# QuentinHuan/ENSEM3A_OpenCLRaytracer

Measured on AMD Instinct MI355X. Metric: Msamples/s Cornell box 1024x1024 64spp; 1/2/4/8-GPU scaling; HBM %peak, higher is better.
Workload: dtype f32; 1 GPU; cornell_1024_s64; scene=cornell, width=1024, height=1024, spp=64, max_bounce=4, traversal=fast, bvh=sah, parallelism=row-interleaved x1

## Files before the change

### ensem3a_openclraytracer_amd/_native.py

```python
from __future__ import annotations

import ctypes
import os
import threading

import numpy as np

from ._build import LIB

_lock = threading.Lock()
_lib = None
_host = None

RT_TRAVERSAL_FAST = 0
RT_TRAVERSAL_REF = 1
RT_BVH_REFERENCE = 0
RT_BVH_SAH = 1
RT_ERR_ARG = 1
RT_ERR_STATE = 3
RT_ACCUM_MAX_SAMPLES = 1 << 24

EXPORTED = (
    "rt_create", "rt_destroy", "rt_last_error", "rt_set_scene", "rt_set_env", "rt_set_option",
    "rt_render", "rt_render_device", "rt_tile_rows", "rt_count_work", "rt_count_work_detail", "rt_work_bytes", "rt_gamma",
    "rt_render_rgb8", "rt_rgb8_device", "rt_rgb8",
    "rt_accum_begin", "rt_accum_add", "rt_accum_add_rgb8", "rt_accum_read", "rt_accum_samples", "rt_accum_end",
    "rt_accum_begin_device", "rt_accum_add_device",
    "rt_accum_mark", "rt_accum_select", "rt_accum_select_mask", "rt_accum_select_all", "rt_accum_selection",
    "rt_accum_sample_map", "rt_accum_add_selected", "rt_accum_mark_device", "rt_accum_select_device",
    "rt_accum_select_mask_device", "rt_accum_select_all_device", "rt_accum_add_selected_device",
    "rt_accum_guides", "rt_accum_guides_device", "rt_denoise_device", "rt_accum_denoise",
    "rt_trace", "rt_trace_device",
    "rt_bvh_build", "rt_device_count", "rt_debug_math", "rt_debug_fn", "rt_debug_trace", "rt_debug_trace_clustered", "rt_debug_scene_info", "rt_debug_pixel_log",
    "rt_debug_wave_counts", "rt_debug_quantise_axis", "rt_debug_timings", "rt_debug_brute_layout",
    "rt_debug_brute_clusters", "rt_debug_brute_shell", "rt_debug_brute_near", "rt_debug_brute_quad",
    "rt_debug_brute_direct", "rt_debug_last_direct", "rt_debug_shell_word",
    "rt_debug_brute_slices",
    "rt_debug_last_slices",
    "rt_debug_brute_refill", "rt_debug_last_refill", "rt_debug_last_launch",
    "rt_obj_parse", "rt_obj_size", "rt_obj_copy", "rt_obj_free", "rt_obj_last_error",
    "rt_scene_check", "rt_scene_last_error",
)
HOST_ONLY = ("rt_bvh_build", "rt_obj_parse", "rt_obj_size", "rt_obj_copy", "rt_obj_free", "rt_obj_last_error",
             "rt_scene_check", "rt_scene_last_error", "rt_debug_quantise_axis", "rt_debug_brute_layout",
             "rt_debug_brute_clusters", "rt_debug_brute_shell", "rt_debug_brute_near", "rt_debug_brute_quad")

_c_p = ctypes.c_void_p
_i64 = ctypes.c_int64
_i32 = ctypes.c_int


class DenoiseParams(ctypes.Structure):
    _fields_ = [("passes", ctypes.c_int), ("normal_squarings", ctypes.c_int),
                ("sigma_c", ctypes.c_float), ("sigma_p", ctypes.c_float)]
# ... 678 lines not shown
    return bool(out[0]), int(out[1]), int(out[2])


def last_slices() -> int:
    return int(lib().rt_debug_last_slices())


def brute_refill(nloc: int, lanes: int, option: int = -1) -> int:
    out = np.zeros(1, np.int32)
    st = lib().rt_debug_brute_refill(int(nloc), int(lanes), int(option), out.ctypes.data)
    if st != 0:
        raise NativeError(st, "rt_debug_brute_refill: bad arguments")
    return int(out[0])


def last_refill():
    out = np.zeros(3, np.int64)
    st = lib().rt_debug_last_refill(out.ctypes.data)
    if st != 0:
        raise NativeError(st, "rt_debug_last_refill: bad arguments")
    return int(out[0]), int(out[1]), int(out[2])


LAUNCH_FIELDS = ("trav", "count", "log", "smem", "ovf", "resume", "step", "wide", "brute", "ts", "acc",
                 "team", "walk_team", "slices", "refill", "grid", "lds", "shell", "near", "quad")
BRUTE_SLICED = 4
BRUTE_REFILL = 8


def last_launch() -> dict:
    out = np.zeros(len(LAUNCH_FIELDS), np.int32)
    st = lib().rt_debug_last_launch(out.ctypes.data)
    if st != 0:
        raise NativeError(st, "rt_debug_last_launch: bad arguments")
    return {name: int(v) for name, v in zip(LAUNCH_FIELDS, out)}


def tile_rows(npix: int, width: int, row0: int, row_step: int) -> int:
    return int(lib().rt_tile_rows(int(npix), int(width), int(row0), int(row_step)))
```

### ensem3a_openclraytracer_amd/csrc/rt_api.hip

```cpp
#include <hip/hip_runtime.h>

#include <cmath>
#include <cstdarg>
#include <cstdio>
#include <algorithm>
#include <array>
#include <atomic>
#include <chrono>
#include <cstring>
#include <map>
#include <string>
#include <thread>
#include <vector>

#include "../../include/rt_api.h"
#include "../../include/rt_debug.h"
#include "rt_internal.h"
#include "scene_pack.h"

constexpr int kResumeMinBvh2 = 36, kResumeMinWide = 48;
constexpr int kDenoiseLds = 1;

using rt::HostScene;

// ... 66 lines not shown
}

struct rt_ctx {
    std::vector<Device> devs;
    HostScene hs;
    bool have_scene = false;
    bool have_env = false;
    int ibl_w = 0, ibl_h = 0;
    int traversal = RT_TRAVERSAL_FAST;
    int bvh_layout = RT_BVH_SAH;
    int brute_max = RT_BRUTE_MAX_DEFAULT;
    int brute_cluster = -1;
    int brute_shell = -1;
    int brute_near = -1;
    int brute_direct = -1;
    int brute_quad = -1;
    int resume_min = -1;
    int team = 0;
    int walk_team = 0;
    int max_waves = 0;
    int step = 0;
    int sun_skip = 1;
    int sun_any = 1;
    int block = 128;
    int bvh_width = 0;
    int fixed_point = 1;
    int sun_cache = 1;
    int pilot = -1;
    int pilot_chunk = 0;
    int pilot_levels = 0;
// ... 144 lines not shown
    s.nmat = ctx->hs.nmat;
    s.ibl_sum = (const uint32_t*)d.ibl_sum.p;
    s.ibl_w = ctx->ibl_w;
    s.ibl_h = ctx->ibl_h;
    s.depth = wide ? std::max(ctx->hs.depth, ctx->hs.wdepth) : ctx->hs.depth;
    s.brute = (const float4*)d.brute.p;
    s.brute_box = (const float4*)d.brute_box.p;
    s.nbrute = ctx->hs.nbrute;
    s.nbox = ctx->hs.nbox;
    s.brute_cbox = (const float4*)d.brute_cbox.p;
    s.brute_crow = (const float4*)d.brute_crow.p;
    s.ncluster = ctx->hs.ncluster;
    s.ncslot = (int32_t)(ctx->hs.brute_cbox.size() / 8);
    s.nsingle4 = s.ncslot - rt::kClusterSlots * s.ncluster;
    s.host_flags = (ctx->brute_cluster < 0 ? rt::kHostClusterAuto : 0) | (ctx->hs.nquad > 0 ? rt::kHostQuad : 0) |
                   (ctx->hs.nshell > 0 && ctx->brute_direct != 0 ? rt::kHostDirect : 0);
    s.nsingle = ctx->hs.nsingle;
    s.shell = ctx->hs.nshell > 0 ? 2 * s.ncslot : 0;
    s.near_floor = s.shell && ctx->brute_near != 0 ? ctx->hs.shell_floor : 0.0f;
    s.near_mask_lo = s.near_floor != 0.0f ? (uint32_t)ctx->hs.shell_mask : 0u;
    s.near_mask_hi = s.near_floor != 0.0f ? (uint32_t)(ctx->hs.shell_mask >> 32) : 0u;
    s.stack_lds = std::min<int32_t>(s.depth > 0 ? s.depth : 1,
                                    ctx->stack_lds > 0 ? ctx->stack_lds : wide ? rt::kStackLdsWide : rt::kStackLds);
    s.stack_ovf = (int2*)d.stack_ovf.p;
    return s;
}

int check_frame(rt_ctx* ctx, const float* cam, const float* env, int64_t npix, int spp, int max_bounce, int row0,
                int row_step, rt::FrameParams* fp) {
    if (!ctx) return set_err(nullptr, RT_ERR_ARG, "null context");
    if (!ctx->have_scene) return set_err(ctx, RT_ERR_STATE, "rt_set_scene has not been called");
// ... 108 lines not shown
};

std::string bounds_message(const char* fmt, int a, int b = 0) {
    char buf[128];
    snprintf(buf, sizeof buf, fmt, a, b);
    return buf;
}

const std::vector<Option>& options() {
    constexpr Effect none = Effect::kNone, invalidate = Effect::kInvalidate, repack = Effect::kRepack;
    static const std::vector<Option> table = {
        {"traversal", &rt_ctx::traversal, range(RT_TRAVERSAL_FAST, RT_TRAVERSAL_REF), "traversal must be 0 (fast) or 1 (ref)", invalidate},
        {"brute_near", &rt_ctx::brute_near, range(-1, 1), "brute_near must be -1 (auto), 0 (off) or 1 (auto)", none},
        {"brute_quad", &rt_ctx::brute_quad, range(-1, 1), "brute_quad must be -1 (auto), 0 (off) or 1 (auto)", repack},
        {"brute_direct", &rt_ctx::brute_direct, range(-1, 1), "brute_direct must be -1 (auto), 0 (off) or 1 (auto)", repack},
        {"bvh", &rt_ctx::bvh_layout, range(RT_BVH_REFERENCE, RT_BVH_SAH), "bvh must be 0 (reference tree) or 1 (sah)", repack},
        {"brute_cluster", &rt_ctx::brute_cluster, range(-1, 1), "brute_cluster must be -1 (auto), 0 (off) or 1 (force)", repack},
        {"brute_shell", &rt_ctx::brute_shell, range(-1, 1), "brute_shell must be -1 (auto), 0 (off) or 1 (force)", repack},
        {"brute_max", &rt_ctx::brute_max, range(0, 4096), "brute_max must be in 0..4096", repack},
        {"resume_min", &rt_ctx::resume_min, range(-1, 64), "resume_min must be -1 (auto) or 0..64", none},
        {"team", &rt_ctx::team, one_of({0, 1, 2, 4, 8}), "team must be 0 (auto), 1, 2, 4 or 8", none},
        {"walk_team", &rt_ctx::walk_team, one_of({0, 1, 2, 4, 8}), "walk_team must be 0 (auto), 1, 2, 4 or 8", none},
        {"sun_any", &rt_ctx::sun_any, range(0, 1), "sun_any must be 0 or 1", none},
        {"sun_skip", &rt_ctx::sun_skip, range(0, 1), "sun_skip must be 0 or 1", none},
        {"step", &rt_ctx::step, range(0, 2), "step must be 0 (auto), 1 (item) or 2 (round)", none},
        {"waves", &rt_ctx::max_waves, range(0, 8), "waves must be in 0..8", none},
        {"pilot", &rt_ctx::pilot, range(-1, 1 << 20), "pilot must be -1 (auto), 0 (off) or a sample count", none},
        {"pilot_chunk", &rt_ctx::pilot_chunk, range(0, 4096), "pilot_chunk must be in 0..4096 (0 = auto)", none},
        {"pilot_levels", &rt_ctx::pilot_levels, zero_or(2, 256), "pilot_levels must be 0 (auto) or 2..256", none},
        {"stack_lds", &rt_ctx::stack_lds, zero_or(kStackLdsMin, rt::kStackLds),
// ... 1266 lines not shown
    const rt::LaunchNote n = rt::last_launch();
    const rt::KernelKey& k = n.key;
    const int64_t v[20] = {k.trav, k.count, k.log,  k.smem,       k.ovf,    k.resume, k.step, k.wide,          k.brute,
                           k.ts,   k.acc,   n.team, n.walk_team,  n.slices, n.refill, n.grid, (int64_t)n.lds,
                           n.shell, n.near, n.quad};
    for (int i = 0; i < 20; ++i) out[i] = (int32_t)std::min<int64_t>(v[i], INT32_MAX);
    return RT_OK;
}

int rt_debug_brute_refill(int64_t nloc, int64_t lanes, int option, int32_t* out) {
    if (!out || nloc < 0 || lanes < 0 || option < -1 || option > rt::kRefillMax) return RT_ERR_ARG;
    *out = rt::brute_refill_launch(option, nloc, lanes);
    return RT_OK;
}

int rt_debug_last_refill(int64_t out[3]) {
    if (!out) return RT_ERR_ARG;
    out[0] = rt::last_launch().refill;
    out[1] = g_refill_events.load(std::memory_order_relaxed);
    out[2] = g_refill_lanes.load(std::memory_order_relaxed);
    return RT_OK;
}

int rt_debug_timings(rt_ctx* ctx, double out[4]) {
    if (!ctx || !out) return set_err(ctx, RT_ERR_ARG, "bad arguments");
    out[0] = ctx->t_pack_ms;
    out[1] = ctx->t_upload_ms;
    out[2] = ctx->t_env_ms;
    out[3] = ctx->t_render_ms;
    return RT_OK;
// ... 17 lines not shown
```

### ensem3a_openclraytracer_amd/csrc/rt_internal.h

```cpp
#pragma once
#include <hip/hip_runtime.h>
#include <cstdint>

#include "rt_layout.h"
#include "rt_slices.h"

namespace rt {

constexpr int32_t kHostClusterAuto = 1;
constexpr int32_t kHostDirect = 4;
constexpr int32_t kHostQuad = 2;
struct DevScene {
    const float4* nodes;
    int32_t nnodes;
    int32_t root_ref;
    const float4* wnodes;
    const float4* wleaves;
    int32_t wroot_ref;
    float wdq_omax;
    float root_box[6];
    const float* bvh9;
    int32_t nbvh9;
    int32_t ref_stack;
    const float4* tri_geo;
    const float4* tri_fast;
    const float4* tri_shade;
// ... 119 lines not shown
    int log;
    int smem;
    int ovf;
    int resume;
    int step;
    int wide;
    int brute;
    int ts;
    int acc;
};
inline bool operator==(const KernelKey& a, const KernelKey& b) {
    return a.trav == b.trav && a.count == b.count && a.log == b.log && a.smem == b.smem && a.ovf == b.ovf &&
           a.resume == b.resume && a.step == b.step && a.wide == b.wide && a.brute == b.brute && a.ts == b.ts &&
           a.acc == b.acc;
}
KernelKey choose_kernel(const DevScene& sc, const FrameParams& fp, int traversal, bool count, bool log, int acc,
                        int block);
int64_t resident_blocks(const void* fn, int block, size_t lds, int max_waves, hipError_t* err);
struct QueryOptions {
    int engine;
    int grid_cap;
    int resume_min;
    int max_waves;
    int block;
};
hipError_t launch_query(const DevScene& sc, int traversal, int any, const float4* rays, float4* out, int64_t n,
                        const QueryOptions& q, unsigned int* counter, hipStream_t stream);
struct LaunchNote {
    KernelKey key;
    int team, walk_team, slices, refill;
// ... 31 lines not shown
```

### ensem3a_openclraytracer_amd/csrc/rt_kernels.hip

```cpp
#include <mutex>
#include <vector>

#include "rt_device.h"

namespace rt {

namespace {

__device__ __forceinline__ void save_state(float4* __restrict__ st, int p, rtm_f3 acc, float kc, uint32_t seed0,
                                           uint32_t seed1, int tc, int s) {
    st[2 * (int64_t)p] = make_float4(acc.x, acc.y, acc.z, kc);
    st[2 * (int64_t)p + 1] =
        make_float4(__uint_as_float(seed0), __uint_as_float(seed1), __int_as_float(tc), __int_as_float(s));
}

[[maybe_unused]] constexpr int kAccAdd = 1;
constexpr int kAccListed = 2;
constexpr int kBruteSliced = 4;
constexpr int kBruteRefill = 8;
template <int TRAV, bool COUNT, bool LOG = false, bool SMEM = false, bool OVF = false, int BRUTE_ = 0, int ACC = 0>
#ifndef RT_RENDER_WAVES
#define RT_RENDER_WAVES 5
#endif
__global__ void __launch_bounds__(256) __attribute__((amdgpu_waves_per_eu(RT_RENDER_WAVES))) render_kernel(DevScene S, FrameParams F, float* __restrict__ out,
                                               unsigned long long* __restrict__ counts,
                                               unsigned int* __restrict__ work_counter,
                                               const LaunchConst* __restrict__ lconst) {
    constexpr int BRUTE = BRUTE_ & 3;
    constexpr bool SLICED = (BRUTE_ & kBruteSliced) != 0;
    static_assert(!SLICED || BRUTE == 1 || BRUTE == 3, "sample slices: the one-lane brute-force loops");
    constexpr bool kRefill = (BRUTE == 1 || BRUTE == 3) && ((BRUTE_ & kBruteRefill) != 0 || COUNT || LOG);
    static_assert(!(BRUTE_ & kBruteRefill) || BRUTE == 1 || BRUTE == 3, "refill threshold: the one-lane brute-force loops");
    extern __shared__ __attribute__((aligned(16))) int lds_stack[];
    const int B = blockDim.x;
    int* stk = lds_stack + threadIdx.x;
    const LaneStack lst = lane_stack(S, lds_stack);
    Cnt c{};
    const float4* mtrec = nullptr;
    const float4* boxrec = nullptr;
    const float4* tshade = S.tri_shade;
    const float4* tframe = S.tri_frame;
    const float* tmat = S.mat;
    constexpr bool ROWS = RT_SHADE_ROWS && (BRUTE == 1 || BRUTE == 3);
    const float4* trow = nullptr;
    if (BRUTE) {
        float4* lr = reinterpret_cast<float4*>(reinterpret_cast<char*>(lds_stack) + (B / 64) * BRUTE_WAVE_LDS);
        float4* ls = lr + 3 * S.nbrute;
// ... 56 lines not shown
    const int W = F.width;
    const int imgSize = (int)F.npix;
    const float e3 = F.env[3], e4 = F.env[4];
    const int spp = F.spp, maxB = F.max_bounce;
    const unsigned int nloc = ACC == kAccListed ? (unsigned int)__builtin_amdgcn_readfirstlane((int)*F.pilot_cost)
                                                : (unsigned int)F.nloc;
    const int lane = threadIdx.x & 63;
    const int ts = BRUTE == 2 ? F.team : 1;
    const int team_lane0 = lane & ~(ts - 1);
    const bool team_leader = lane == team_lane0;
    const unsigned long long team_leaders = ts == 1 ? ~0ull : ts == 2 ? 0x5555555555555555ull
                                             : ts == 4 ? 0x1111111111111111ull : 0x0101010101010101ull;

    int phase = FETCH;
    PixelQueue pq;
    pq.per = (F.handout && F.pass != 2) ? (unsigned)(((ACC == kAccListed ? (int64_t)nloc : F.nloc) + kGroups - 1) / kGroups) : 0u;
    if constexpr (kRefill) pq.dry = F.refill > 1 ? (unsigned)min(F.refill, 64) << kQueueRefillShift : 0u;
    int p = 0, i = 0;
    bool logme = false;
    uint32_t seed0 = 0, seed1 = 0;
    rtm_f3 cd = rtm_v3(0, 0, 0);
    float kc = 1000.0f;
    int tc = -1;
    rtm_f3 so = rtm_v3(1, 1, 1);
    float k = 1000.0f;
    int tri = -1, j = 0;
    rtm_f3 Bo = rtm_v3(0, 0, 0), Bd = rtm_v3(0, 0, 0);
    rtm_f3 acc = rtm_v3(0, 0, 0);
    int s = 0;
    [[maybe_unused]] int plim = 0;
    auto slimit = [&]() __attribute__((always_inline)) { if constexpr (ACC == kAccListed) return plim; else return spp; };
// ... 39 lines not shown
        }
        if (need) {
            unsigned sl = kWholeJob;
            unsigned int q;
            if constexpr (SLICED) q = take_job<kRefill>(pq, need, team_lane0, work_counter, nloc, lane, nsl, stail, sl);
            else q = take_pixel<kRefill>(pq, need, team_lane0, work_counter, nloc, lane);
            if (SLICED && phase == FETCH && q < nloc && sl != kWholeJob && sl > 0) {
                p = (int)q;
                lim = (int)sl;
                s = send(sl - 1u);
                phase = WAIT_SLICE;
            } else if (phase == FETCH) {
                const bool whole = !SLICED || sl == kWholeJob;
                bool ok = q < nloc;
                if (ok) {
                    p = (ACC == kAccListed || F.pass == 2) ? (int)F.pilot_order[q] : (int)q;
                    const int krow = p / W;
                    const int col = p - krow * W;
                    const int64_t i64 = ((int64_t)F.row0 + (int64_t)krow * F.row_step) * W + col;
                    ok = i64 < F.npix;
                    i = (int)i64;
                }
                if (ok) {
                    if constexpr (SLICED) {
                        seed0 = (uint32_t)i;
                        seed1 = 0;
                    } else {
                        seed0 = (uint32_t)(i % imgSize);
                        seed1 = (uint32_t)(i / imgSize);
                    }
                    cd = camera_dir(C, W, i);
                    acc = rtm_v3(0, 0, 0);
                    s = 0;
                    cost = 0;
                    sun0 = -2;
                    phase = PRIMARY;
                    logme = LOG && i == F.log_pixel;
                    if (F.pass == 2) {
                        const float4 a = F.pilot_state[2 * (int64_t)p], b = F.pilot_state[2 * (int64_t)p + 1];
                        acc = rtm_v3(a.x, a.y, a.z);
                        kc = a.w;
                        seed0 = __float_as_uint(b.x);
                        seed1 = __float_as_uint(b.y);
                        tc = __float_as_int(b.z);
                        s = __float_as_int(b.w);
                        tri = tc; j = 0;
                        so = rtm_v3(1, 1, 1);
                        phase = s >= spp ? FETCH : PREP;
                    }
                    if constexpr (ACC) if (ACC == kAccListed || F.pilot > 0) {
                        const float4 a = F.pilot_state[2 * (int64_t)p], b = F.pilot_state[2 * (int64_t)p + 1];
                        acc = rtm_v3(a.x, a.y, a.z);
                        kc = a.w;
// ... 25 lines not shown
                so = rtm_v3(1, 1, 1);
                lim = send((unsigned)lim);
                phase = s >= spp ? FETCH : PREP;
            }
        }
        if (__all(phase == DONE)) break;
        if (SLICED && __all(phase == DONE || phase == WAIT_SLICE)) __builtin_amdgcn_s_sleep(8);
        if (COUNT && lane == 0) c.wave_outer++;
        if (phase == DONE || phase == FETCH || (SLICED && phase == WAIT_SLICE)) continue;

        if (phase == PREP) {
            bool done = true;
            const bool cam = j == 0;
            const rtm_f3 Ro = cam ? C.position : Bo, Rd = cam ? cd : Bd;
            const float kh = cam ? kc : k;
            if (j > maxB) {
            } else if (tri < 0) {
                so = rtm_scale(rtm_mul(so, sample_ibl_if<COUNT>(S, C, Rd, e4, c)), e4);
            } else {
                const float4 sh = ROWS ? trow[2 * tri] : tshade[tri];
                const rtm_f3 n = xyz(sh);
                const Mat cm = ROWS ? row_mat(sh, trow[2 * tri + 1]) : load_mat(tmat, __float_as_int(sh.w));
                if (cm.type == 0) {
                    so = rtm_scale(so, cm.rough);
                } else {
                    const float4 f2 = tframe[3 * tri + 2];
                    const rtm_f3 nn = xyz(f2);
                    float invPdf = 0.0f;
                    rtm_f3 brdf = rtm_v3(0, 0, 0);
                    if (COUNT) count_event(c, cm.type);
                    if (cm.type == 1) {
// ... 10 lines not shown
                        invPdf = 1.0f / rtm_fabs(rtm_dot(Bd, nn));
                    }
                    const rtm_f3 nd = dev_normalize(Rd);
                    Bo = rtm_v3(fmaf(nd.x, kh, Ro.x), fmaf(nd.y, kh, Ro.y), fmaf(nd.z, kh, Ro.z));
                    const float att = invPdf * rtm_fabs(rtm_dot(Bd, nn));
                    so = rtm_scale(rtm_mul(so, brdf), att);
                    phase = BOUNCE;
                    done = false;
                }
            }
            if (done) {
                if (LOG && logme) log_event(F, 3.0f, s + 1, rtm_v3(0, 0, 0), rtm_v3(0, 0, 0), 0.0f, 0, so);
                acc = rtm_add(acc, so);
                if (COUNT) c.samples++;
                ++s;
                if (TRAV == TRAV_FAST && F.fixed_point && j == 0 && !(LOG && logme)) {
                    if (COUNT) c.samples += (unsigned long long)max(slimit() - s, 0);
                    for (; s < slimit(); ++s) acc = rtm_add(acc, so);
                }
                if (s >= slimit()) {
                    phase = FETCH;
                    if (team_leader) store_pixel(out, p, acc, slimit());
                    if (F.pass == 1) save_pilot();
                    if constexpr (ACC) { if (team_leader) save_state(F.pilot_state, p, acc, kc, seed0, seed1, tc, s); }
                    if constexpr (SLICED) { if (lim < spp) save_slice(cd); }
                } else if (F.pass == 1 && s >= F.pilot) {
                    save_pilot();
                    phase = FETCH;
                } else if (SLICED && s >= lim) {
                    save_slice(cd);
                    phase = FETCH;
                } else {
                    tri = tc; j = 0;
                    so = rtm_v3(1, 1, 1);
                }
                continue;
            }
        }

        const rtm_f3 to = (phase == PRIMARY) ? C.position : Bo;
        const rtm_f3 td = (phase == PRIMARY) ? cd : ((phase == BOUNCE) ? Bd : C.sun);
// ... 1 lines not shown
        if constexpr (STAMPS) chain_stamp(stamp_wl, kStampHead);
        const Hit h = trace<TRAV, COUNT, SMEM, OVF, BRUTE != 0, BRUTE == 3>(S, nodes, tris, to, td, stk, B, lst, c, mtrec, ts, boxrec);
        if (COUNT && lane == __ffsll((long long)__ballot(1)) - 1) {
            const unsigned long long dt = clock64() - t_tr;
            c.cyc_trav += dt;
            c.cyc_shade -= dt;
        }
        ++cost;
        bool finish = false;
        if (phase == PRIMARY) {
            tc = h.tri;
            kc = h.k;
            tri = tc; j = 0;
            so = rtm_v3(1, 1, 1);
            phase = PREP;
            if (spp <= 0) {
                if (team_leader) store_pixel(out, p, acc, spp);
                phase = FETCH;
            }
            continue;
        }
        if (LOG && logme) {
            const int hm = h.tri >= 0 ? __float_as_int(S.tri_shade[h.tri].w) : 0;
            log_event(F, phase == BOUNCE ? 1.0f : 2.0f, j, Bo, td, h.tri >= 0 ? h.k : -1.0f, hm, so);
        }
        int sun_hit = -2;
        const bool sun_first = TRAV == TRAV_FAST && F.sun_cache && j == 0 && !(LOG && logme);
        if (phase == BOUNCE) {
            if (h.tri >= 0) {
                tri = h.tri; k = h.k;
                const Mat bm = ROWS ? row_mat(trow[2 * h.tri], trow[2 * h.tri + 1])
                                    : load_mat(tmat, __float_as_int(tshade[h.tri].w));
                if (bm.type != 0) {
                    if (j == maxB) {
                        so = rtm_v3(0, 0, 0);
                        finish = true;
                    } else {
                        ++j;
                        phase = PREP;
                    }
                } else {
                    so = rtm_scale(so, bm.rough);
                    finish = true;
                }
            } else if (TRAV == TRAV_FAST && F.sun_skip) {
                sun_hit = -1;
            } else if (sun_first && sun0 != -2) {
                sun_hit = sun0;
            } else {
                phase = SUN;
            }
        } else {
            sun_hit = h.tri;
            if (sun_first) sun0 = h.tri;
        }
        if (sun_hit != -2) {
            rtm_f3 sunLight = rtm_v3(0, 0, 0);
            if (COUNT) c.sun++;
            const Mat cm = ROWS ? row_mat(trow[2 * tri], trow[2 * tri + 1])
                                : load_mat(tmat, __float_as_int(tshade[tri].w));
            if (sun_hit < 0 && cm.type != 3) sunLight = rtm_v3(e3, e3, e3);
            if (sun_hit >= 0) {
                const Mat sm = ROWS ? row_mat(trow[2 * sun_hit], trow[2 * sun_hit + 1])
                                    : load_mat(tmat, __float_as_int(tshade[sun_hit].w));
                if (sm.type == 3) sunLight = rtm_scale(sm.color, e3);
            }
            const rtm_f3 envLight = rtm_scale(sample_ibl_if<COUNT>(S, C, Bd, e4, c), e4);
            so = rtm_mul(so, rtm_add(sunLight, envLight));
            finish = true;
        }
        if (finish) {
            if (LOG && logme) log_event(F, 3.0f, s + 1, rtm_v3(0, 0, 0), rtm_v3(0, 0, 0), 0.0f, 0, so);
            acc = rtm_add(acc, so);
            if (COUNT) c.samples++;
            ++s;
            if (s >= slimit()) {
                if (team_leader) store_pixel(out, p, acc, slimit());
                if (F.pass == 1) save_pilot();
                if constexpr (ACC) { if (team_leader) save_state(F.pilot_state, p, acc, kc, seed0, seed1, tc, s); }
                phase = FETCH;
            } else if (F.pass == 1 && s >= F.pilot) {
                save_pilot();
                phase = FETCH;
            } else if (SLICED && s >= lim) {
                save_slice(cd);
                phase = FETCH;
            } else {
                tri = tc; j = 0;
                so = rtm_v3(1, 1, 1);
                phase = PREP;
            }
        }
    }
    if constexpr (STAMPS) {
        if ((threadIdx.x & 63) == 0 && counts) {
            const unsigned long long* st = reinterpret_cast<const unsigned long long*>(stamp_wl + BRUTE_STAMP_OFF);
// ... 502 lines not shown
    t.push_back(walk_row<COUNT, false, true, false, false, 0, 1>());
    t.push_back(walk_row<COUNT, false, false, true, false, 0, 1>());
    t.push_back(walk_row<COUNT, false, false, false, false, 0, 1>());
    t.push_back(render_row<TRAV_FAST, COUNT, false, false, false, 1>());
    if constexpr (!COUNT) t.push_back(render_row<TRAV_FAST, COUNT, false, false, false, 3>());
    t.push_back(render_row<TRAV_FAST, COUNT, false, false, false, 2>());
    if constexpr (!COUNT) t.push_back(render_row<TRAV_FAST, COUNT, false, false, false, 3 | kBruteSliced>());
    t.push_back(render_row<TRAV_FAST, COUNT, false, false, false, 1 | kBruteSliced>());
    if constexpr (!COUNT) {
        t.push_back(render_row<TRAV_FAST, COUNT, false, false, false, 3 | kBruteSliced | kBruteRefill>());
        t.push_back(render_row<TRAV_FAST, COUNT, false, false, false, 1 | kBruteSliced | kBruteRefill>());
        t.push_back(render_row<TRAV_FAST, COUNT, false, false, false, 3 | kBruteRefill>());
        t.push_back(render_row<TRAV_FAST, COUNT, false, false, false, 1 | kBruteRefill>());
    }
}

__global__ void debug_math_kernel(int fn, const float* __restrict__ x, const float* __restrict__ y,
                                  float* __restrict__ out, int64_t n) {
    const int64_t i = (int64_t)blockIdx.x * blockDim.x + threadIdx.x;
    if (i >= n) return;
    float r = 0.0f;
    switch (fn) {
        case 0: r = rtm_sin(x[i]); break;
        case 1: r = rtm_cos(x[i]); break;
        case 2: r = rtm_tan(x[i]); break;
        case 3: r = rtm_asin(x[i]); break;
        case 4: r = rtm_acos(x[i]); break;
        case 5: r = rtm_atan2(x[i], y[i]); break;
        case 6: r = sqrtf(x[i]); break;
        case 7: r = x[i] / y[i]; break;
// ... 161 lines not shown
#endif

namespace {
const void* kernel_fn(const KernelKey& k) {
    static const std::vector<KernelRow> table = [] {
        std::vector<KernelRow> t;
#ifndef RT_ACCUM_TU
        log_rows(t);
        head_rows<true>(t);
        head_rows<false>(t);
        engine_rows<true>(t);
#else
        head_rows<false>(t);
#endif
        engine_rows<false>(t);
        return t;
    }();
    for (const KernelRow& r : table)
        if (r.key == k) return r.fn;
    return nullptr;
}

hipError_t launch_pick(const DevScene& sc, const FrameParams& fp, KernelKey k, int block, float* d_out,
                       unsigned long long* d_counts, unsigned int* d_work, hipStream_t stream) {
    if (fp.nloc <= 0) return hipSuccess;
    const bool brute = k.brute != 0, product = !k.count && !k.log, listed = k.acc == kAccListed;
    size_t lds = (brute ? brute_lds_bytes(sc, block, true) : stack_lds_bytes(sc, k.trav, block)) +
                 (k.smem ? staged_scene_bytes(sc) : 0);
    hipError_t e = hipSuccess;
    auto resident = [&](int max_waves) { return resident_blocks(kernel_fn(k), block, lds, max_waves, &e); };
// ... 5 lines not shown
    if (brute && !listed && fp.pass == 0 && fp.team <= 1 && fp.slice_state && fp.slice_ready &&
        sc.ntri + 2 < 65536 && fp.npix <= INT_MAX)
        bslices = brute_slice_launch(fp.slices, fp.nloc, lanes);
    if (!k.resume) f.slices = bslices;
    f.team = !brute ? 1 : bslices ? 1 : fp.team;
    if (f.team == 0) f.team = (!listed && fp.nloc * 4 <= lanes) ? 4 : 1;
    f.walk_team = 1;
    if (k.resume && k.step && !k.wide && !k.log) {
        f.walk_team = fp.walk_team ? fp.walk_team : listed ? 1 : auto_walk_team(fp.nloc, lanes);
        if (f.walk_team != 2 && f.walk_team != 4 && f.walk_team != 8) f.walk_team = 1;
    }
    f.refill = (brute && f.team <= 1) ? brute_refill_launch(fp.refill, fp.nloc, lanes) : 0;
    k.ts = f.walk_team;
    if (brute && f.team > 1) k.brute = 2;
    else if (brute) k.brute |= (bslices ? kBruteSliced : 0) | (product && f.refill > 1 ? kBruteRefill : 0);
    if (brute && f.team <= 1) lds = brute_lds_bytes(sc, block, false);
    const void* fn = kernel_fn(k);
    const int64_t need = (fp.nloc * f.team * f.walk_team + block - 1) / block;
    const int64_t grid = std::min(need, resident(fp.max_waves));
    if (e != hipSuccess) return e;
    if (bslices) e = hipMemsetAsync(f.slice_ready, 0, (size_t)fp.nloc * sizeof(uint32_t), stream);
    const LaunchConst* lc = nullptr;
    if (e == hipSuccess) e = setup_work_block(f, d_work, stream, &lc);
    if (e != hipSuccess) return e;
    const int shell = (k.brute & 3) == 3 && sc.shell != 0;
    note_launch({k, f.team, f.walk_team, f.slices, f.refill, grid, lds, shell, shell && sc.near_floor != 0.0f,
                 shell && (sc.host_flags & kHostQuad) != 0, shell && (sc.host_flags & kHostDirect) != 0});
#if RT_CHAIN_STAMPS
    if (!d_counts) d_counts = chain_stamp_buffer();
#endif
// ... 424 lines not shown
```

### ensem3a_openclraytracer_amd/csrc/scene_pack.cpp

```cpp
#include "scene_pack.h"

#include <algorithm>
#include <array>
#include <cmath>
#include <cstdarg>
#include <cstdio>
#include <cstring>
#include <atomic>
#include <functional>
#include <map>
#include <mutex>
#include <new>
#include <stdexcept>
#include <string>
#include <system_error>
#include <thread>
#include <vector>

#include "../../include/rt_api.h"
#include "../../include/rt_debug.h"
#include "../../include/rt_scene.h"
#include "bvh_sah.h"

using rt::HostScene;
// ... 826 lines not shown
    emit_bvh(hs, L.data(), R.data(), T.data(), box.data(), nn);
    return true;
}

}

namespace rt {

bool shell_direct(HostScene& hs, int direct) {
    if (hs.nshell <= 0 || hs.brute_shell.size() < (size_t)rt::kShellRecF) return false;
    const int32_t w = as_i32(hs.brute_shell[7]);
    hs.brute_shell[7] = as_f32(direct != 0 ? (w | rt::kShellDirect) : (w & ~rt::kShellDirect));
    return direct != 0;
}

void pack_checked(HostScene& hs, const float* bvh9, int64_t nb, int64_t ntri, int layout, int brute_max, int cluster,
                  int shell, int quad, std::string& why) {
    hs.fast_ok = (ntri > 0) ? pack_fast(hs, bvh9, nb, ntri, layout, brute_max, cluster, shell, quad, why) : true;
    if (hs.fast_ok && ntri > 0) {
        double m1 = 0.0, m2 = 0.0;
        for (int64_t t = 0; t < ntri; ++t) {
            const float* g = hs.tri_geo.data() + 12 * t;
            const double l1 = std::sqrt((double)g[4] * g[4] + (double)g[5] * g[5] + (double)g[6] * g[6]);
            const double l2 = std::sqrt((double)g[8] * g[8] + (double)g[9] * g[9] + (double)g[10] * g[10]);
            if (std::isfinite(l1)) m1 = std::max(m1, l1);
            if (std::isfinite(l2)) m2 = std::max(m2, l2);
        }
        if (!(m1 * m2 <= std::ldexp(1.0, 120))) {
            hs.fast_ok = false;
            why = "triangle edges beyond 2^60 (the FAST reciprocal needs |e1 . (d x e2)| <= 2^126)";
// ... 38 lines not shown
    for (int64_t m = 0; m < M; ++m) {
        const float tf = mat[6 * m];
        if (!(tf > -1.0f && tf < 4.0f))
            return fail(msg, RT_ERR_SCENE, "material %lld has type %g; the kernel defines types 0..3", (long long)m,
                           (double)tf);
    }
    hs.ntri = (int32_t)T;
    hs.nmat = (int32_t)M;
    hs.nbvh9 = (int32_t)NB;
    hs.mat.assign((size_t)rt::kMatF * M, 0.0f);
    for (int64_t m = 0; m < M; ++m) {
        for (int k = 0; k < 6; ++k) hs.mat[(size_t)rt::kMatF * m + k] = mat[6 * m + k];
        for (int k = 1; k < 4; ++k) hs.colors_finite = hs.colors_finite && std::isfinite(mat[6 * m + k]);
        hs.has_glass = hs.has_glass || (int)mat[6 * m] == 3;
    }
    if (bvh9) hs.bvh9.assign(bvh9, bvh9 + nbvh);
    hs.tri_geo.assign((size_t)T * 12, 0.0f);
    hs.tri_shade.assign((size_t)T * 4, 0.0f);
    for (int64_t t = 0; t < T; ++t) {
        const int32_t* f = face + 10 * t;
        if (f[0] < 0 || f[0] >= M)
            return fail(msg, RT_ERR_ARG, "triangle %lld: material %d out of range [0,%lld)", (long long)t, f[0],
                           (long long)M);
        for (int j = 7; j < 10; ++j)
            if (f[j] < 0 || f[j] >= NV)
                return fail(msg, RT_ERR_ARG, "triangle %lld: position index %d out of range", (long long)t, f[j]);
        if (f[4] < 0 || f[4] >= NN)
            return fail(msg, RT_ERR_ARG, "triangle %lld: normal index %d out of range", (long long)t, f[4]);
        const float* a = vp + 3 * (int64_t)f[7];
        const float* b = vp + 3 * (int64_t)f[8];
// ... 284 lines not shown
```

### ensem3a_openclraytracer_amd/csrc/scene_pack.h

```cpp
#pragma once
#include <cstdint>
#include <string>
#include <vector>

#include "rt_layout.h"

namespace rt {

struct HostScene {
    std::vector<float> nodes;
    std::vector<float> wnodes;
    std::vector<float> wleaves;
    int32_t nwnodes = 0, wroot_ref = 0, wdepth = 1;
    float wdq_omax = 0.0f;
    std::vector<float> bvh9;
    std::vector<float> tri_geo;
    std::vector<float> tri_fast;
    std::vector<float> tri_shade;
    std::vector<float> mat;
    std::vector<float> brute;
    std::vector<float> brute_box;
    int32_t nbrute = 0;
    int32_t nbox = 0;
    std::vector<float> brute_cbox;
    std::vector<float> brute_crow;
    int32_t ncluster = 0, nsingle = 0;
    std::vector<float> brute_shell;
    int32_t nshell = 0, nrest = 0;
    int32_t nquad = 0;
    std::vector<uint8_t> brute_near;
    float shell_floor = 0.0f;
    uint64_t shell_mask = 0;
    int32_t nnodes = 0, root_ref = 0, ntri = 0, nmat = 0, nbvh9 = 0, depth = 1;
    float root_box[6] = {0, 0, 0, 0, 0, 0};
    bool fast_ok = false;
    bool colors_finite = true;
    bool has_glass = false;
};


int scene_prepare(HostScene& hs, const float* vp, int64_t nvp, const float* vn, int64_t nvn, const int32_t* face,
                  int64_t nface, const float* mat, int64_t nmat, const float* bvh9, int64_t nbvh, int layout,
                  int brute_max, int cluster, int shell, int quad, std::string& msg, std::string& why);

void pack_checked(HostScene& hs, const float* bvh9, int64_t nb, int64_t ntri, int layout, int brute_max, int cluster,
                  int shell, int quad, std::string& why);

bool shell_direct(HostScene& hs, int direct);

}
```

### include/rt_debug.h

```cpp
#ifndef RT_DEBUG_H
#define RT_DEBUG_H

#include <stdint.h>
#include "rt_api.h"


#ifdef __cplusplus
extern "C" {
#endif

int rt_debug_math(rt_ctx* ctx, int fn, const float* x, const float* y, float* out, int64_t n);

int rt_debug_trace(rt_ctx* ctx, int traversal, const float* rays, float* out, int64_t n);

int rt_debug_trace_clustered(rt_ctx* ctx, const float* rays, float* out, int64_t n, int32_t info[4]);

enum {
    RT_FN_CAMERA = 0, RT_FN_SUN = 1, RT_FN_HEMI = 2, RT_FN_GGX = 3, RT_FN_IBL = 4, RT_FN_MT_REF = 5,
    RT_FN_MT_FAST = 6, RT_FN_BOX_REF = 7, RT_FN_BOX_FAST = 8, RT_FN_COUNT = 9
};
int rt_debug_fn(rt_ctx* ctx, int fn, const float* in, float* out, int64_t n);

int rt_debug_pixel_log(rt_ctx* ctx, int traversal, const float cam[10], const float env[5], int64_t npix, int spp,
                       int max_bounce, int64_t pixel, float* log, int cap, int* n_events, float out3[3]);
// ... 35 lines not shown

int rt_debug_last_direct(void);

int rt_debug_shell_word(rt_ctx* ctx);

int rt_debug_brute_slices(int64_t nloc, int64_t lanes, int spp, int option, int accum_base, int32_t out[3]);

int rt_debug_last_slices(void);

int rt_debug_last_launch(int32_t out[20]);

int rt_debug_brute_refill(int64_t nloc, int64_t lanes, int option, int32_t* out);

int rt_debug_last_refill(int64_t out[3]);

#ifdef __cplusplus
}
#endif
#endif
```

Before: 12610 Msamples/s.

## Add lean brute-force kernel variant for diffuse-only scenes without IBL

Adds a compile-time LEAN flag to the one-lane brute-force render kernels, selected automatically when every material is diffuse or emissive, the environment-map weight is zero, and no pilot or accumulation passes are in use. The lean path skips IBL sampling, pilot-order indirection and pilot state saves, and most material loads, and reads the material type and colour straight from the row data. This cuts per-bounce work and register pressure but adds more kernel instantiations. It also relies on the host-side material classification to be correct for it to be safe.

```diff
diff --git a/ensem3a_openclraytracer_amd/_native.py b/ensem3a_openclraytracer_amd/_native.py
--- a/ensem3a_openclraytracer_amd/_native.py
+++ b/ensem3a_openclraytracer_amd/_native.py
@@ -37,7 +37,7 @@
     "rt_debug_brute_direct", "rt_debug_last_direct", "rt_debug_shell_word",
     "rt_debug_brute_slices",
     "rt_debug_last_slices",
-    "rt_debug_brute_refill", "rt_debug_last_refill", "rt_debug_last_launch",
+    "rt_debug_brute_refill", "rt_debug_last_refill", "rt_debug_last_launch", "rt_debug_brute_lean",
     "rt_obj_parse", "rt_obj_size", "rt_obj_copy", "rt_obj_free", "rt_obj_last_error",
     "rt_scene_check", "rt_scene_last_error",
 )
@@ -746,6 +746,21 @@
     return int(out[0])
 
 
+def brute_lean(materialData, env, spp: int = 4, max_bounce: int = 4, pass_: int = 0, pilot: int = 0,
+               fixed_point: int = 1, sun_cache: int = 1, option: int = -1, loop: int = 3, team: int = 1,
+               count: int = 0, log: int = 0, acc: int = 0, traversal: int = 0):
+    mat, e = f32(materialData), f32(env)
+    fn = lib().rt_debug_brute_lean
+    fn.restype, fn.argtypes = _i32, [_c_p, _i64, _c_p, _c_p, _c_p, _c_p]
+    frame = np.array([spp, max_bounce, pass_, pilot, fixed_point, sun_cache, option], np.int32)
+    kernel = np.array([loop, team, count, log, acc, traversal], np.int32)
+    out = np.zeros(2, np.int32)
+    st = fn(ptr(mat) if mat.size else None, mat.size, ptr(e), frame.ctypes.data, kernel.ctypes.data, out.ctypes.data)
+    if st != 0:
+        raise NativeError(st, "rt_debug_brute_lean: bad arguments")
+    return bool(out[0]), bool(out[1])
+
+
 def last_refill():
     out = np.zeros(3, np.int64)
     st = lib().rt_debug_last_refill(out.ctypes.data)
@@ -758,6 +773,7 @@
                  "team", "walk_team", "slices", "refill", "grid", "lds", "shell", "near", "quad")
 BRUTE_SLICED = 4
 BRUTE_REFILL = 8
+BRUTE_LEAN = 16
 
 
 def last_launch() -> dict:
diff --git a/ensem3a_openclraytracer_amd/csrc/rt_api.hip b/ensem3a_openclraytracer_amd/csrc/rt_api.hip
--- a/ensem3a_openclraytracer_amd/csrc/rt_api.hip
+++ b/ensem3a_openclraytracer_amd/csrc/rt_api.hip
@@ -104,6 +104,7 @@
     int brute_shell = -1;
     int brute_near = -1;
     int brute_direct = -1;
+    int brute_lean = -1;
     int brute_quad = -1;
     int resume_min = -1;
     int team = 0;
@@ -278,7 +279,8 @@
     s.ncslot = (int32_t)(ctx->hs.brute_cbox.size() / 8);
     s.nsingle4 = s.ncslot - rt::kClusterSlots * s.ncluster;
     s.host_flags = (ctx->brute_cluster < 0 ? rt::kHostClusterAuto : 0) | (ctx->hs.nquad > 0 ? rt::kHostQuad : 0) |
-                   (ctx->hs.nshell > 0 && ctx->brute_direct != 0 ? rt::kHostDirect : 0);
+                   (ctx->hs.nshell > 0 && ctx->brute_direct != 0 ? rt::kHostDirect : 0) |
+                   (ctx->hs.diffuse_only && ctx->brute_lean != 0 ? rt::kHostLean : 0);
     s.nsingle = ctx->hs.nsingle;
     s.shell = ctx->hs.nshell > 0 ? 2 * s.ncslot : 0;
     s.near_floor = s.shell && ctx->brute_near != 0 ? ctx->hs.shell_floor : 0.0f;
@@ -417,6 +419,7 @@
         {"brute_near", &rt_ctx::brute_near, range(-1, 1), "brute_near must be -1 (auto), 0 (off) or 1 (auto)", none},
         {"brute_quad", &rt_ctx::brute_quad, range(-1, 1), "brute_quad must be -1 (auto), 0 (off) or 1 (auto)", repack},
         {"brute_direct", &rt_ctx::brute_direct, range(-1, 1), "brute_direct must be -1 (auto), 0 (off) or 1 (auto)", repack},
+        {"brute_lean", &rt_ctx::brute_lean, range(-1, 1), "brute_lean must be -1 (auto), 0 (off) or 1 (auto)", none},
         {"bvh", &rt_ctx::bvh_layout, range(RT_BVH_REFERENCE, RT_BVH_SAH), "bvh must be 0 (reference tree) or 1 (sah)", repack},
         {"brute_cluster", &rt_ctx::brute_cluster, range(-1, 1), "brute_cluster must be -1 (auto), 0 (off) or 1 (force)", repack},
         {"brute_shell", &rt_ctx::brute_shell, range(-1, 1), "brute_shell must be -1 (auto), 0 (off) or 1 (force)", repack},
@@ -1713,6 +1716,24 @@
     return RT_OK;
 }
 
+int rt_debug_brute_lean(const float* mat, int64_t nmat6, const float env[5], const int32_t frame[7],
+                        const int32_t kernel[6], int32_t out[2]) {
+    if ((nmat6 > 0 && !mat) || nmat6 < 0 || nmat6 % 6 || !env || !frame || !kernel || !out) return RT_ERR_ARG;
+    if (frame[6] < -1 || frame[6] > 1) return RT_ERR_ARG;
+    out[0] = rt::materials_diffuse_only(mat, nmat6) ? 1 : 0;
+    rt::FrameParams fp{};
+    std::memcpy(fp.env, env, sizeof fp.env);
+    fp.spp = frame[0];
+    fp.max_bounce = frame[1];
+    fp.pass = frame[2];
+    fp.pilot = frame[3];
+    fp.fixed_point = frame[4];
+    fp.sun_cache = frame[4] && frame[5] ? 1 : 0;
+    rt::KernelKey k{kernel[5], kernel[2], kernel[3], 0, 0, 0, 1, 0, kernel[0], 1, kernel[4]};
+    out[1] = rt::brute_lean_kernel(k, kernel[1]) && rt::brute_lean_frame(out[0] && frame[6] != 0 ? rt::kHostLean : 0, fp);
+    return RT_OK;
+}
+
 int rt_debug_last_refill(int64_t out[3]) {
     if (!out) return RT_ERR_ARG;
     out[0] = rt::last_launch().refill;
diff --git a/ensem3a_openclraytracer_amd/csrc/rt_internal.h b/ensem3a_openclraytracer_amd/csrc/rt_internal.h
--- a/ensem3a_openclraytracer_amd/csrc/rt_internal.h
+++ b/ensem3a_openclraytracer_amd/csrc/rt_internal.h
@@ -1,6 +1,7 @@
 #pragma once
 #include <hip/hip_runtime.h>
 #include <cstdint>
+#include <cstring>
 
 #include "rt_layout.h"
 #include "rt_slices.h"
@@ -10,6 +11,7 @@
 constexpr int32_t kHostClusterAuto = 1;
 constexpr int32_t kHostDirect = 4;
 constexpr int32_t kHostQuad = 2;
+constexpr int32_t kHostLean = 8;
 struct DevScene {
     const float4* nodes;
     int32_t nnodes;
@@ -159,6 +161,16 @@
            a.resume == b.resume && a.step == b.step && a.wide == b.wide && a.brute == b.brute && a.ts == b.ts &&
            a.acc == b.acc;
 }
+constexpr int kBruteLean = 16;
+inline bool brute_lean_frame(int32_t host_flags, const FrameParams& fp) {
+    uint32_t e4;
+    std::memcpy(&e4, &fp.env[4], sizeof e4);
+    return (host_flags & kHostLean) != 0 && e4 == 0u && fp.pass == 0 && fp.pilot == 0 && fp.spp > 0 &&
+           fp.max_bounce >= 0 && fp.fixed_point != 0 && fp.sun_cache != 0;
+}
+inline bool brute_lean_kernel(const KernelKey& k, int team) {
+    return (k.brute & 3) != 0 && (k.brute & 3) != 2 && team <= 1 && k.trav == 0 && !k.count && !k.log && !k.acc && !k.resume;
+}
 KernelKey choose_kernel(const DevScene& sc, const FrameParams& fp, int traversal, bool count, bool log, int acc,
                         int block);
 int64_t resident_blocks(const void* fn, int block, size_t lds, int max_waves, hipError_t* err);
diff --git a/ensem3a_openclraytracer_amd/csrc/rt_kernels.hip b/ensem3a_openclraytracer_amd/csrc/rt_kernels.hip
--- a/ensem3a_openclraytracer_amd/csrc/rt_kernels.hip
+++ b/ensem3a_openclraytracer_amd/csrc/rt_kernels.hip
@@ -31,6 +31,9 @@
     static_assert(!SLICED || BRUTE == 1 || BRUTE == 3, "sample slices: the one-lane brute-force loops");
     constexpr bool kRefill = (BRUTE == 1 || BRUTE == 3) && ((BRUTE_ & kBruteRefill) != 0 || COUNT || LOG);
     static_assert(!(BRUTE_ & kBruteRefill) || BRUTE == 1 || BRUTE == 3, "refill threshold: the one-lane brute-force loops");
+    constexpr bool LEAN = (BRUTE_ & kBruteLean) != 0;
+    static_assert(!LEAN || ((BRUTE == 1 || BRUTE == 3) && TRAV == TRAV_FAST && !COUNT && !LOG && !ACC && RT_SHADE_ROWS),
+                  "lean: the one-lane one-shot product kernels");
     extern __shared__ __attribute__((aligned(16))) int lds_stack[];
     const int B = blockDim.x;
     int* stk = lds_stack + threadIdx.x;
@@ -117,7 +120,7 @@
 
     int phase = FETCH;
     PixelQueue pq;
-    pq.per = (F.handout && F.pass != 2) ? (unsigned)(((ACC == kAccListed ? (int64_t)nloc : F.nloc) + kGroups - 1) / kGroups) : 0u;
+    pq.per = (F.handout && (LEAN || F.pass != 2)) ? (unsigned)(((ACC == kAccListed ? (int64_t)nloc : F.nloc) + kGroups - 1) / kGroups) : 0u;
     if constexpr (kRefill) pq.dry = F.refill > 1 ? (unsigned)min(F.refill, 64) << kQueueRefillShift : 0u;
     int p = 0, i = 0;
     bool logme = false;
@@ -187,7 +190,8 @@
                 const bool whole = !SLICED || sl == kWholeJob;
                 bool ok = q < nloc;
                 if (ok) {
-                    p = (ACC == kAccListed || F.pass == 2) ? (int)F.pilot_order[q] : (int)q;
+                    if constexpr (LEAN) p = (int)q;
+                    else p = (ACC == kAccListed || F.pass == 2) ? (int)F.pilot_order[q] : (int)q;
                     const int krow = p / W;
                     const int col = p - krow * W;
                     const int64_t i64 = ((int64_t)F.row0 + (int64_t)krow * F.row_step) * W + col;
@@ -209,7 +213,7 @@
                     sun0 = -2;
                     phase = PRIMARY;
                     logme = LOG && i == F.log_pixel;
-                    if (F.pass == 2) {
+                    if (!LEAN && F.pass == 2) {
                         const float4 a = F.pilot_state[2 * (int64_t)p], b = F.pilot_state[2 * (int64_t)p + 1];
                         acc = rtm_v3(a.x, a.y, a.z);
                         kc = a.w;
@@ -265,7 +269,28 @@
             const bool cam = j == 0;
             const rtm_f3 Ro = cam ? C.position : Bo, Rd = cam ? cd : Bd;
             const float kh = cam ? kc : k;
-            if (j > maxB) {
+            if constexpr (LEAN) {
+                if (tri < 0) {
+                    so = rtm_mul(so, rtm_v3(0.0f, 0.0f, 0.0f));
+                } else {
+                    const float4 sh = trow[2 * tri], r1 = trow[2 * tri + 1];
+                    if ((int)sh.w == 0) {
+                        so = rtm_scale(so, r1.w);
+                    } else {
+                        const float4 f2 = tframe[3 * tri + 2];
+                        const rtm_f3 nn = xyz(f2);
+                        float invPdf = 0.0f;
+                        Bd = hemi_cosine(xyz(sh), tframe[3 * tri], tframe[3 * tri + 1], f2, &seed1, &seed0, &invPdf);
+                        const rtm_f3 brdf = rtm_scale(rtm_v3(r1.x, r1.y, r1.z), 1.0f / 3.14f);
+                        const rtm_f3 nd = dev_normalize(Rd);
+                        Bo = rtm_v3(fmaf(nd.x, kh, Ro.x), fmaf(nd.y, kh, Ro.y), fmaf(nd.z, kh, Ro.z));
+                        const float att = invPdf * rtm_fabs(rtm_dot(Bd, nn));
+                        so = rtm_scale(rtm_mul(so, brdf), att);
+                        phase = BOUNCE;
+                        done = false;
+                    }
+                }
+            } else if (j > maxB) {
             } else if (tri < 0) {
                 so = rtm_scale(rtm_mul(so, sample_ibl_if<COUNT>(S, C, Rd, e4, c)), e4);
             } else {
@@ -306,17 +331,17 @@
                 acc = rtm_add(acc, so);
                 if (COUNT) c.samples++;
                 ++s;
-                if (TRAV == TRAV_FAST && F.fixed_point && j == 0 && !(LOG && logme)) {
+                if (TRAV == TRAV_FAST && (LEAN || F.fixed_point) && j == 0 && !(LOG && logme)) {
                     if (COUNT) c.samples += (unsigned long long)max(slimit() - s, 0);
                     for (; s < slimit(); ++s) acc = rtm_add(acc, so);
                 }
                 if (s >= slimit()) {
                     phase = FETCH;
                     if (team_leader) store_pixel(out, p, acc, slimit());
-                    if (F.pass == 1) save_pilot();
+                    if (!LEAN && F.pass == 1) save_pilot();
                     if constexpr (ACC) { if (team_leader) save_state(F.pilot_state, p, acc, kc, seed0, seed1, tc, s); }
                     if constexpr (SLICED) { if (lim < spp) save_slice(cd); }
-                } else if (F.pass == 1 && s >= F.pilot) {
+                } else if (!LEAN && F.pass == 1 && s >= F.pilot) {
                     save_pilot();
                     phase = FETCH;
                 } else if (SLICED && s >= lim) {
@@ -348,7 +373,7 @@
             tri = tc; j = 0;
             so = rtm_v3(1, 1, 1);
             phase = PREP;
-            if (spp <= 0) {
+            if (!LEAN && spp <= 0) {
                 if (team_leader) store_pixel(out, p, acc, spp);
                 phase = FETCH;
             }
@@ -359,12 +384,13 @@
             log_event(F, phase == BOUNCE ? 1.0f : 2.0f, j, Bo, td, h.tri >= 0 ? h.k : -1.0f, hm, so);
         }
         int sun_hit = -2;
-        const bool sun_first = TRAV == TRAV_FAST && F.sun_cache && j == 0 && !(LOG && logme);
+        const bool sun_first = TRAV == TRAV_FAST && (LEAN || F.sun_cache) && j == 0 && !(LOG && logme);
         if (phase == BOUNCE) {
             if (h.tri >= 0) {
                 tri = h.tri; k = h.k;
-                const Mat bm = ROWS ? row_mat(trow[2 * h.tri], trow[2 * h.tri + 1])
-                                    : load_mat(tmat, __float_as_int(tshade[h.tri].w));
+                const Mat bm = LEAN ? Mat{(int)trow[2 * h.tri].w, rtm_v3(0, 0, 0), 0.0f}
+                               : ROWS ? row_mat(trow[2 * h.tri], trow[2 * h.tri + 1])
+                                      : load_mat(tmat, __float_as_int(tshade[h.tri].w));
                 if (bm.type != 0) {
                     if (j == maxB) {
                         so = rtm_v3(0, 0, 0);
@@ -374,7 +400,7 @@
                         phase = PREP;
                     }
                 } else {
-                    so = rtm_scale(so, bm.rough);
+                    so = rtm_scale(so, LEAN ? trow[2 * h.tri + 1].w : bm.rough);
                     finish = true;
                 }
             } else if (TRAV == TRAV_FAST && F.sun_skip) {
@@ -389,18 +415,23 @@
             if (sun_first) sun0 = h.tri;
         }
         if (sun_hit != -2) {
-            rtm_f3 sunLight = rtm_v3(0, 0, 0);
             if (COUNT) c.sun++;
-            const Mat cm = ROWS ? row_mat(trow[2 * tri], trow[2 * tri + 1])
-                                : load_mat(tmat, __float_as_int(tshade[tri].w));
-            if (sun_hit < 0 && cm.type != 3) sunLight = rtm_v3(e3, e3, e3);
-            if (sun_hit >= 0) {
-                const Mat sm = ROWS ? row_mat(trow[2 * sun_hit], trow[2 * sun_hit + 1])
-                                    : load_mat(tmat, __float_as_int(tshade[sun_hit].w));
-                if (sm.type == 3) sunLight = rtm_scale(sm.color, e3);
+            if constexpr (LEAN) {
+                const float l = (sun_hit < 0 ? e3 : 0.0f) + 0.0f;
+                so = rtm_mul(so, rtm_v3(l, l, l));
+            } else {
+                rtm_f3 sunLight = rtm_v3(0, 0, 0);
+                const Mat cm = ROWS ? row_mat(trow[2 * tri], trow[2 * tri + 1])
+                                    : load_mat(tmat, __float_as_int(tshade[tri].w));
+                if (sun_hit < 0 && cm.type != 3) sunLight = rtm_v3(e3, e3, e3);
+                if (sun_hit >= 0) {
+                    const Mat sm = ROWS ? row_mat(trow[2 * sun_hit], trow[2 * sun_hit + 1])
+                                        : load_mat(tmat, __float_as_int(tshade[sun_hit].w));
+                    if (sm.type == 3) sunLight = rtm_scale(sm.color, e3);
+                }
+                const rtm_f3 envLight = rtm_scale(sample_ibl_if<COUNT>(S, C, Bd, e4, c), e4);
+                so = rtm_mul(so, rtm_add(sunLight, envLight));
             }
-            const rtm_f3 envLight = rtm_scale(sample_ibl_if<COUNT>(S, C, Bd, e4, c), e4);
-            so = rtm_mul(so, rtm_add(sunLight, envLight));
             finish = true;
         }
         if (finish) {
@@ -410,10 +441,10 @@
             ++s;
             if (s >= slimit()) {
                 if (team_leader) store_pixel(out, p, acc, slimit());
-                if (F.pass == 1) save_pilot();
+                if (!LEAN && F.pass == 1) save_pilot();
                 if constexpr (ACC) { if (team_leader) save_state(F.pilot_state, p, acc, kc, seed0, seed1, tc, s); }
                 phase = FETCH;
-            } else if (F.pass == 1 && s >= F.pilot) {
+            } else if (!LEAN && F.pass == 1 && s >= F.pilot) {
                 save_pilot();
                 phase = FETCH;
             } else if (SLICED && s >= lim) {
@@ -946,6 +977,15 @@
         t.push_back(render_row<TRAV_FAST, COUNT, false, false, false, 1 | kBruteRefill>());
     }
 }
+template <int LOOP>
+void lean_rows(std::vector<KernelRow>& t) {
+    if constexpr (RT_SHADE_ROWS && !kTuAcc) {
+        t.push_back(render_row<TRAV_FAST, false, false, false, false, LOOP | kBruteLean>());
+        t.push_back(render_row<TRAV_FAST, false, false, false, false, LOOP | kBruteSliced | kBruteLean>());
+        t.push_back(render_row<TRAV_FAST, false, false, false, false, LOOP | kBruteSliced | kBruteRefill | kBruteLean>());
+        t.push_back(render_row<TRAV_FAST, false, false, false, false, LOOP | kBruteRefill | kBruteLean>());
+    }
+}
 
 __global__ void debug_math_kernel(int fn, const float* __restrict__ x, const float* __restrict__ y,
                                   float* __restrict__ out, int64_t n) {
@@ -1137,6 +1177,8 @@
         head_rows<false>(t);
 #endif
         engine_rows<false>(t);
+        lean_rows<3>(t);
+        lean_rows<1>(t);
         return t;
     }();
     for (const KernelRow& r : table)
@@ -1172,6 +1214,7 @@
     k.ts = f.walk_team;
     if (brute && f.team > 1) k.brute = 2;
     else if (brute) k.brute |= (bslices ? kBruteSliced : 0) | (product && f.refill > 1 ? kBruteRefill : 0);
+    if (RT_SHADE_ROWS && !kTuAcc && brute_lean_kernel(k, f.team) && brute_lean_frame(sc.host_flags, f)) k.brute |= kBruteLean;
     if (brute && f.team <= 1) lds = brute_lds_bytes(sc, block, false);
     const void* fn = kernel_fn(k);
     const int64_t need = (fp.nloc * f.team * f.walk_team + block - 1) / block;
diff --git a/ensem3a_openclraytracer_amd/csrc/scene_pack.cpp b/ensem3a_openclraytracer_amd/csrc/scene_pack.cpp
--- a/ensem3a_openclraytracer_amd/csrc/scene_pack.cpp
+++ b/ensem3a_openclraytracer_amd/csrc/scene_pack.cpp
@@ -864,6 +864,12 @@
     return direct != 0;
 }
 
+bool materials_diffuse_only(const float* mat, int64_t nmat6) {
+    for (int64_t m = 0; m < nmat6 / 6; ++m)
+        if (!(mat[6 * m] > -1.0f && mat[6 * m] < 2.0f)) return false;
+    return true;
+}
+
 void pack_checked(HostScene& hs, const float* bvh9, int64_t nb, int64_t ntri, int layout, int brute_max, int cluster,
                   int shell, int quad, std::string& why) {
     hs.fast_ok = (ntri > 0) ? pack_fast(hs, bvh9, nb, ntri, layout, brute_max, cluster, shell, quad, why) : true;
@@ -932,6 +938,7 @@
         for (int k = 1; k < 4; ++k) hs.colors_finite = hs.colors_finite && std::isfinite(mat[6 * m + k]);
         hs.has_glass = hs.has_glass || (int)mat[6 * m] == 3;
     }
+    hs.diffuse_only = materials_diffuse_only(mat, nmat);
     if (bvh9) hs.bvh9.assign(bvh9, bvh9 + nbvh);
     hs.tri_geo.assign((size_t)T * 12, 0.0f);
     hs.tri_shade.assign((size_t)T * 4, 0.0f);
diff --git a/ensem3a_openclraytracer_amd/csrc/scene_pack.h b/ensem3a_openclraytracer_amd/csrc/scene_pack.h
--- a/ensem3a_openclraytracer_amd/csrc/scene_pack.h
+++ b/ensem3a_openclraytracer_amd/csrc/scene_pack.h
@@ -36,7 +36,10 @@
     bool fast_ok = false;
     bool colors_finite = true;
     bool has_glass = false;
+    bool diffuse_only = true;
 };
+
+bool materials_diffuse_only(const float* mat, int64_t nmat6);
 
 
 int scene_prepare(HostScene& hs, const float* vp, int64_t nvp, const float* vn, int64_t nvn, const int32_t* face,
diff --git a/include/rt_debug.h b/include/rt_debug.h
--- a/include/rt_debug.h
+++ b/include/rt_debug.h
@@ -73,6 +73,9 @@
 
 int rt_debug_last_refill(int64_t out[3]);
 
+int rt_debug_brute_lean(const float* materialData, int64_t n_mat, const float env[5], const int32_t frame[7],
+                        const int32_t kernel[6], int32_t out[2]);
+
 #ifdef __cplusplus
 }
 #endif
```

After: 13050 Msamples/s (median of 6 runs). +3.5%, better.
